# uzh-rpg/rpg_svo

Measured on AMD Instinct MI355X. Metric: frames/sec sparse-align+pose-refine (VGA, 4 pyr lvls); ATE vs CPU ref, higher is better.
Workload: dtype value = default build: K1 f32 pixels/residuals/chi2/per-pixel products, f64 Jacobian rows/partials/reductions/projection/solve/pose; K4 f64 (reference-width build: roofline_f64_build.value)

## Files before the change

include/svo_hip.h:

```cpp
#ifndef SVO_HIP_H_
#define SVO_HIP_H_

#include <stddef.h>
#include <stdint.h>

#ifdef __cplusplus
extern "C" {
#endif

#define SVO_HIP_MAX_LEVELS 8
#define SVO_HIP_STORE_TAIL_PAD 256
#define SVO_HIP_MAX_PATCHES 1024

#define SVO_HIP_OK 0
#define SVO_HIP_EINVAL (-1)
#define SVO_HIP_ERANGE (-2)
#define SVO_HIP_EHIP (-3)
#define SVO_HIP_ENODEV (-4)
#define SVO_HIP_ENOMEM (-5)

#define SVO_HIP_HALFSAMPLE_SCALAR 0
#define SVO_HIP_HALFSAMPLE_SSE2 1
#define SVO_HIP_HALFSAMPLE_AUTO 2

// ... 225 lines not shown
  int32_t* d_visit_cell;
  int32_t* d_visit_trial;
  int32_t* d_trial_cur;
  double* d_trial_pos;
  int32_t* d_trial_obs_begin;
  int32_t* d_trial_obs_end;
  int32_t* d_trial_cell;
  double* d_trial_px;
} svo_hip_reprojection;

int svo_hip_reproject_map(const svo_hip_camera* cam, const svo_hip_frames* frames, int cur_frame,
                          const int32_t* d_kf_rank, const svo_hip_map* map, const svo_hip_map_patch* patch,
                          const svo_hip_grid* grid, int first_cell, int max_cells_with_trials, int max_visits,
                          int max_trials, const svo_hip_reprojection* out, void* stream);

int svo_hip_find_match_direct_indirect(const svo_hip_pyr_layout* layout, const uint8_t* d_store,
                                       const svo_hip_camera* cam, const svo_hip_frames* frames, int M_cap,
                                       const int32_t* d_M, const int32_t* d_cur_frame, const double* d_pt_pos,
                                       const int32_t* d_obs_begin, const int32_t* d_obs_end,
                                       const svo_hip_features* obs, int n_pyr_levels, int align_max_iter,
                                       double* d_px_cur, int32_t* d_ok, int32_t* d_ref_obs, int32_t* d_search_level,
                                       double* d_A_cur_ref, uint8_t* d_patch_out, void* d_workspace,
                                       size_t workspace_bytes, void* stream);
int svo_hip_select_matches_indirect(const svo_hip_camera* cam, int M_cap, const int32_t* d_M, const int32_t* d_cell,
                                    const int32_t* d_ok, const double* d_px, const int32_t* d_level,
                                    const double* d_pos, int max_fts, int32_t* d_n, int32_t* d_sel, double* d_f,
                                    int32_t* d_level_out, double* d_pos_out, uint8_t* d_has_point, int32_t* d_signal,
                                    int32_t signal_value, void* stream);

int svo_hip_compose_poses(int n, const double* d_A, const double* d_B, double* d_out,
                          const int32_t* d_out_index, void* stream);
int svo_hip_cam2world(const svo_hip_camera* cam, int n, const double* d_px, double* d_f,
                      void* stream);
int svo_hip_frame_pose_compose(const double* d_T_cur_ref, const double* d_q_ref, const double* d_t_ref, double* d_frame_T,
                               int cur_frame, double* d_T_copy, double* d_T_out, const svo_hip_camera* cam, int n_frames,
                               int n_kf, const double* d_key_pos, const uint8_t* d_key_valid, int max_n_kfs, int32_t* d_rank,
                               int32_t* d_rank_out, int32_t* d_signal, int32_t signal_value, void* stream);

int svo_hip_pose_optimize(const svo_hip_camera* cam, int B, const int32_t* d_n, int n_stride,
                          const double* d_f, const int32_t* d_level, const double* d_pos,
                          uint8_t* d_has_point, double reproj_thresh, int n_iter,
                          double* d_T_f_w, double* d_Cov, double* d_stats, int32_t* d_ran,
                          void* stream);
int svo_hip_pose_optimize_ordered(const svo_hip_camera* cam, int B, const int32_t* d_n, int n_stride,
                                  const double* d_f, const int32_t* d_level, const double* d_pos,
                                  uint8_t* d_has_point, double reproj_thresh, int n_iter,
                                  double* d_T_f_w, double* d_Cov, double* d_stats, int32_t* d_ran,
                                  void* stream);

int svo_hip_pose_optimize_deferred(const svo_hip_camera* cam, int B, const int32_t* d_n, int n_stride,
                                   const double* d_f, const int32_t* d_level, const double* d_pos,
                                   uint8_t* d_has_point, double reproj_thresh, int n_iter, double* d_T_f_w,
                                   double* d_Cov, double* d_stats, int32_t* d_ran, void* stream);

int svo_hip_point_optimize(const svo_hip_frames* frames, int P, const int32_t* d_obs_ptr,
                           const int32_t* d_obs_frame, const double* d_obs_f, int n_iter,
                           double* d_pos, void* stream);

typedef struct svo_hip_seeds {
  float* d_a;
  float* d_b;
  float* d_mu;
  float* d_z_range;
  float* d_sigma2;
  const int32_t* d_batch_id;
} svo_hip_seeds;

#define SVO_HIP_SEED_ERASED_OLD 1
#define SVO_HIP_SEED_BEHIND 2
#define SVO_HIP_SEED_NOT_IN_FRAME 3
#define SVO_HIP_SEED_NO_MATCH 4
#define SVO_HIP_SEED_UPDATED 5
#define SVO_HIP_SEED_CONVERGED 6
#define SVO_HIP_SEED_NAN 7

typedef struct svo_hip_depth_filter_options {
  int32_t max_n_kfs;
  int32_t batch_counter;
  double seed_convergence_sigma2_thresh;
  int32_t align_1d;
  int32_t align_max_iter;
  int32_t max_epi_search_steps;
  int32_t subpix_refinement;
  int32_t epi_search_edgelet_filtering;
  int32_t n_pyr_levels;
  double epi_search_edgelet_max_angle;
} svo_hip_depth_filter_options;

int svo_hip_update_seeds(const svo_hip_pyr_layout* layout, const uint8_t* d_store,
                         const svo_hip_camera* cam, const svo_hip_frames* frames, int S,
                         const int32_t* d_cur_frame, const svo_hip_features* ftr,
                         const svo_hip_seeds* seeds, const svo_hip_depth_filter_options* opt,
                         int32_t* d_status, double* d_xyz_world, double* d_px_cur,
                         void* d_workspace, size_t workspace_bytes, void* stream);

typedef struct svo_hip_seed_patch {
  int32_t n;
  int32_t reserved;
  const int32_t* d_slot;
  svo_hip_features src_ftr;
  svo_hip_seeds src_seeds;
} svo_hip_seed_patch;
int svo_hip_seed_store_patch(const svo_hip_seed_patch* patch, const svo_hip_features* store_ftr,
                             const svo_hip_seeds* store_seeds, void* stream);
int svo_hip_update_seeds_resident(const svo_hip_pyr_layout* layout, const uint8_t* d_store,
                                  const svo_hip_camera* cam, const svo_hip_frames* frames, int cur_frame, int S,
// ... 184 lines not shown
```

rpg_svo_amd/capi.py:

```python
from __future__ import annotations

import ctypes as C
import os

MAX_LEVELS = 8
STORE_TAIL_PAD = 256
MAX_PATCHES = 1024

HALFSAMPLE_SCALAR, HALFSAMPLE_SSE2, HALFSAMPLE_AUTO = 0, 1, 2
SIA_STOP = 1

_LIB_PATH = os.environ.get("SVO_HIP_LIB") or os.path.join(os.path.dirname(os.path.abspath(__file__)), "lib", "libsvo_hip.so")


class SvoHipError(RuntimeError):
    pass


class PyrLayout(C.Structure):
    _fields_ = [
        ("n_levels", C.c_int32),
        ("w", C.c_int32 * MAX_LEVELS),
        ("h", C.c_int32 * MAX_LEVELS),
        ("pitch", C.c_int32 * MAX_LEVELS),
# ... 156 lines not shown
    "svo_hip_event_sync": (_i, [_vp]),
    "svo_hip_event_query": (_i, [_vp]),
    "svo_hip_stream_wait_event": (_i, [_vp, _vp]),
    "svo_hip_graph_begin_capture": (_i, [_vp]),
    "svo_hip_graph_end_capture": (_i, [_vp, C.POINTER(_vp)]),
    "svo_hip_graph_launch": (_i, [_vp, _vp]),
    "svo_hip_graph_destroy": (_i, [_vp]),
    "svo_hip_camera_pinhole": (_i, [_i, _i] + [C.c_double] * 9 + [C.POINTER(Camera)]),
    "svo_hip_camera_atan": (_i, [_i, _i] + [C.c_double] * 5 + [C.POINTER(Camera)]),
    "svo_hip_pyr_layout_init": (_i, [_i, _i, _i, C.POINTER(PyrLayout)]),
    "svo_hip_pyr_store_bytes": (_i64, [C.POINTER(PyrLayout), _i]),
    "svo_hip_pyramid_load_level0": (_i, [C.POINTER(PyrLayout), _vp, _i, _i, _vp, _i64, _i, _vp]),
    "svo_hip_pyramid_upload_level0": (_i, [C.POINTER(PyrLayout), _vp, _i, _vp, _i, _vp, _vp]),
    "svo_hip_pyramid_upload_level": (_i, [C.POINTER(PyrLayout), _vp, _i, _i, _vp, _i, _vp, _vp]),
    "svo_hip_pyramid_upload_build": (_i, [C.POINTER(PyrLayout), _vp, _i, _vp, _i, _i, _vp, _vp]),
    "svo_hip_pyramid_build": (_i, [C.POINTER(PyrLayout), _vp, _i, _i, _i, _vp]),
    "svo_hip_pyramid_build_from_images": (_i, [C.POINTER(PyrLayout), _vp, _i, _i, _vp, _i64, _i, _i, _vp]),
    "svo_hip_pyramid_build_tiled": (_i, [C.POINTER(PyrLayout), _vp, _i, _i, _vp, _i64, _i, _i, _i, _vp]),
    "svo_hip_pyramid_build_per_level": (_i, [C.POINTER(PyrLayout), _vp, _i, _i, _i, _vp]),
    "svo_hip_pyramid_download_level": (_i, [C.POINTER(PyrLayout), _vp, _i, _i, _vp, _vp]),
    "svo_hip_sparse_align": (_i, [C.POINTER(PyrLayout), _vp, _i, _vp, _vp, _vp, _i, _vp, _vp, _vp,
                                  C.POINTER(SiaParams), _vp, _vp, _vp, _vp, _vp, _vp, _vp, _vp]),
    "svo_hip_sparse_align_workgroup": (_i, [C.POINTER(PyrLayout), _vp, _i, _vp, _vp, _vp, _i, _vp, _vp, _vp,
                                            C.POINTER(SiaParams), _vp, _vp, _vp, _vp, _vp, _vp, _vp, _vp]),
    "svo_hip_solve6_hipsolver_workspace_bytes": (C.c_size_t, [_i]),
    "svo_hip_solve6_hipsolver": (_i, [_i, _vp, _vp, _vp, _vp, _vp, C.c_size_t, _vp]),
    "svo_hip_align_batch": (_i, [_LP, _vp, _i, _vp, _vp, _vp, _vp, _vp, _i, _vp, _vp, _vp, _vp]),
    "svo_hip_align_batch_counted": (_i, [_LP, _vp, _i, _vp, _vp, _vp, _vp, _vp, _i, _vp, _vp, _vp, _vp, _vp]),
    "svo_hip_align_workspace_bytes": (C.c_size_t, [_i]),
    "svo_hip_align_batch_phased": (_i, [_LP, _vp, _i, _vp, _vp, _vp, _vp, _vp, _i, _vp, _vp, _vp, _vp, _vp, C.c_size_t, _vp]),
    "svo_hip_update_seeds_scan_steps": (_vp, [_vp]),
    "svo_hip_update_seeds_count_evaluations": (C.c_int, [C.c_int]),
    "svo_hip_update_seeds_align_evaluations": (_vp, [_vp, C.c_int]),
    "svo_hip_match_workspace_bytes": (C.c_size_t, [_i]),
    "svo_hip_find_match_direct": (_i, [_LP, _vp, C.POINTER(Camera), C.POINTER(Frames), _i, _vp, _vp, _vp,
                                       C.POINTER(Features), _i, _i, _vp, _vp, _vp, _vp, _vp, _vp, _vp, C.c_size_t, _vp]),
    "svo_hip_reproject_map": (_i, [C.POINTER(Camera), C.POINTER(Frames), _i, _vp, C.POINTER(Map), C.POINTER(MapPatch),
                                   C.POINTER(Grid), _i, _i, _i, _i, C.POINTER(Reprojection), _vp]),
    "svo_hip_find_match_direct_indirect": (_i, [_LP, _vp, C.POINTER(Camera), C.POINTER(Frames), _i, _vp, _vp, _vp, _vp, _vp,
                                                C.POINTER(Features), _i, _i, _vp, _vp, _vp, _vp, _vp, _vp, _vp, C.c_size_t, _vp]),
    "svo_hip_select_matches_indirect": (_i, [C.POINTER(Camera), _i, _vp, _vp, _vp, _vp, _vp, _vp, _i, _vp, _vp, _vp, _vp, _vp,
                                             _vp, _vp, _i, _vp]),
    "svo_hip_reproject_points": (_i, [C.POINTER(Camera), C.POINTER(Frames), _i, _vp, _vp, _i, _i, _vp, _vp, _vp]),
    "svo_hip_compose_poses": (_i, [_i, _vp, _vp, _vp, _vp, _vp]),
    "svo_hip_frame_pose_compose": (_i, [_vp, _vp, _vp, _vp, _i, _vp, _vp, _vp, _i, _i, _vp, _vp, _i, _vp, _vp, _vp, _i, _vp]),
    "svo_hip_cam2world": (_i, [C.POINTER(Camera), _i, _vp, _vp, _vp]),
    "svo_hip_select_matches": (_i, [C.POINTER(Camera), _i, _vp, _vp, _vp, _vp, _vp, _i, _vp, _vp, _vp, _vp, _vp, _vp, _vp, _i, _vp]),
    "svo_hip_pose_optimize": (_i, [C.POINTER(Camera), _i, _vp, _i, _vp, _vp, _vp, _vp, C.c_double, _i, _vp, _vp, _vp,
                                   _vp, _vp]),
    "svo_hip_pose_optimize_ordered": (_i, [C.POINTER(Camera), _i, _vp, _i, _vp, _vp, _vp, _vp, C.c_double, _i, _vp, _vp,
                                           _vp, _vp, _vp]),
    "svo_hip_pose_optimize_deferred": (_i, [C.POINTER(Camera), _i, _vp, _i, _vp, _vp, _vp, _vp, C.c_double, _i, _vp, _vp,
                                           _vp, _vp, _vp]),
    "svo_hip_point_optimize": (_i, [C.POINTER(Frames), _i, _vp, _vp, _vp, _i, _vp, _vp]),
    "svo_hip_update_seeds": (_i, [_LP, _vp, C.POINTER(Camera), C.POINTER(Frames), _i, _vp, C.POINTER(Features),
                                  C.POINTER(Seeds), C.POINTER(DepthFilterOptions), _vp, _vp, _vp, _vp, C.c_size_t, _vp]),
    "svo_hip_seed_store_patch": (_i, [C.POINTER(SeedPatch), C.POINTER(Features), C.POINTER(Seeds), _vp]),
    "svo_hip_update_seeds_resident": (_i, [_LP, _vp, C.POINTER(Camera), C.POINTER(Frames), _i, _i, _vp, C.POINTER(Features),
                                           C.POINTER(Seeds), C.POINTER(DepthFilterOptions), _vp, _vp, _vp, _vp, _vp, C.c_size_t, _vp]),
    "svo_hip_update_seeds_resident_pose": (_i, [_LP, _vp, C.POINTER(Camera), C.POINTER(Frames), _i, _vp, _i, _vp, C.POINTER(Features),
                                                C.POINTER(Seeds), C.POINTER(DepthFilterOptions), _vp, _vp, _vp, _vp, _vp, C.c_size_t, _vp]),
    "svo_hip_find_epipolar_match_direct": (_i, [_LP, _vp, C.POINTER(Camera), C.POINTER(Frames), _i, _vp, C.POINTER(Features),
                                                _vp, _vp, _vp, C.POINTER(DepthFilterOptions), _vp, _vp, _vp, _vp, _vp, C.c_size_t, _vp]),
    "svo_hip_update_seed_batch": (_i, [_i, _vp, _vp, C.POINTER(Seeds), _vp]),
    "svo_hip_fast_workspace_bytes": (C.c_size_t, [_LP, _i, _i]),
    "svo_hip_fast_detect": (_i, [_LP, _vp, _i, _vp, _i, _i, _i, _i, _i, _vp, C.c_double, _vp, _vp, _vp, _vp, C.c_size_t, _vp]),
    "svo_hip_klt_params_default": (_i, [C.POINTER(KltParams)]),
    "svo_hip_klt_track": (_i, [_LP, _vp, _i, _vp, _vp, _i, _vp, _vp, _vp, _vp, C.POINTER(KltParams), _vp]),
    "svo_hip_klt_summarize": (_i, [C.POINTER(Camera), _i, _i, _vp, _vp, _vp, _vp, _vp, _vp, _vp, _vp]),
    "svo_hip_homography_params_default": (_i, [C.POINTER(HomographyParams)]),
    "svo_hip_homography_init": (_i, [C.POINTER(Camera), _i, _i, _vp, _vp, _vp, _vp, _vp, _vp, C.POINTER(HomographyParams),
                                     C.POINTER(HomographyOut), _vp]),
    "svo_hip_first_map": (_i, [C.POINTER(Camera), _i, _i, _vp, _vp, _vp, _vp, _vp, _vp, _vp, _vp, _vp, _i, _i, _i, _i,
                               C.POINTER(FirstMapOut), _vp]),
    "svo_hip_initialize_seeds": (_i, [C.POINTER(Camera), _i, _i, _vp, _vp, _vp, C.c_double, _vp, _vp, _vp, _i, _i,
                                      C.POINTER(SeedInitOut), _vp]),
    "svo_hip_frame_close_params_default": (_i, [C.POINTER(FrameCloseParams)]),
    "svo_hip_frame_close": (_i, [C.POINTER(Camera), _i, _i, _i, C.POINTER(FrameCloseIn), _i, _i, _i, _i, C.POINTER(FrameCloseParams),
                                 C.POINTER(FrameCloseOut), _vp]),
    "svo_hip_compute_tau_batch": (_i, [_i, _vp, _vp, _vp, C.c_double, _vp, _vp]),
}

_lib = None


def lib_path() -> str:
    return _LIB_PATH


def load() -> C.CDLL:
    global _lib
    if _lib is not None:
        return _lib
    if not os.path.exists(_LIB_PATH):
        raise SvoHipError(
            f"{_LIB_PATH} not found: build it with `python -c 'import __graft_entry__ as g; g.build()'` "
            "(hipcc --offload-arch=gfx950).  There is no CPU fallback.")
    import torch
    lib = C.CDLL(_LIB_PATH)
    for name, (res, args) in PROTOTYPES.items():
        fn = getattr(lib, name)
        fn.restype = res
        fn.argtypes = args
    _lib = lib
    return lib

# ... 34 lines not shown
```

rpg_svo_amd/csrc/pose_optimizer.hip:

```cpp
#pragma clang fp contract(off)
#include "track_kernels.h"
#include "track_math.h"

using namespace svo_capi;
using namespace svo_dev;

namespace {

constexpr int PO_MINW = 4;
constexpr int PO_HALF = 32;
constexpr int PO_BLOCK = 64;
constexpr int PO_MAXN = 1024;
constexpr double SVO_EPS = 0.0000000001;

struct PoseArgs {
  Cam cam;
  const int32_t* n;
  int n_stride;
  const double* f;
  const int32_t* level;
  const double* pos;
  uint8_t* has_point;
  double reproj_thresh;
  int n_iter;
  double* T;
  double* Cov;
  double* stats;
  int32_t* ran;
  int only_flagged;
};

struct PoseLds {
  double tile[28][PO_HALF];
  unsigned long long live[PO_BLOCK / 64];
  double acc[28];
  double dT[6];
  double new_chi2;
  Se3 T, T_old;
  double scale;
  double median_d;
  double chi2;
  float median_f;
  int n_err;
  int flag;
};

__device__ __forceinline__ float tukey_weight(float x) {
  const float b_square = 4.6851f * 4.6851f;
  const float x_square = x * x;
  if (x_square <= b_square) {
    const float tmp = 1.0f - x_square / b_square;
    return tmp * tmp;
  }
  return 0.0f;
}

template <typename T>
__device__ __forceinline__ void rank_select(const T* v, int n, int k, T* out) {
  for (int i = threadIdx.x; i < n; i += PO_BLOCK) {
    const T mine = v[i];
    if (!(mine < (T)INFINITY)) continue;
    int rank = 0;
#pragma unroll 8
    for (int j = 0; j < n; ++j) {
      const T o = v[j];
      rank += (o < mine || (o == mine && j < i)) ? 1 : 0;
    }
    if (rank == k) *out = mine;
  }
}

struct PoseDyn {
  double* vals;
  float* err;
  uint8_t* hp;
};

__global__ void __launch_bounds__(PO_BLOCK, PO_MINW) pose_opt_kernel(const PoseArgs a) {
  __shared__ PoseLds s;
  SVO_DYNAMIC_LDS(double, po_dyn);
  const int ns8 = (a.n_stride + 7) & ~7;
  PoseDyn d;
  d.vals = po_dyn;
  d.err = reinterpret_cast<float*>(po_dyn + ns8);
  d.hp = reinterpret_cast<uint8_t*>(d.err + ns8);
  const int b = blockIdx.x;
  const int tid = threadIdx.x;
  if (a.only_flagged && a.ran[b] != 2) return;
  int n = a.n[b];
  n = n < 0 ? 0 : (n > a.n_stride ? a.n_stride : n);
  const size_t base = (size_t)b * a.n_stride;
  const double focal = fabs(a.cam.fx);

  if (tid == 0) {
    se3_from_Rt(a.T + 12 * b, s.T);
    s.T_old = s.T;
    s.n_err = 0;
    s.flag = 0;
    s.chi2 = 0.0;
  }
  for (int i = tid; i < n; i += PO_BLOCK) d.hp[i] = a.has_point[base + i];
  __syncthreads();
  {
    const Se3 T = s.T;
    int cnt = 0;
    for (int i = tid; i < n; i += PO_BLOCK) {
      d.err[i] = INFINITY;
      if (!d.hp[i]) continue;
      const double p[3] = {a.pos[3 * (base + i)], a.pos[3 * (base + i) + 1], a.pos[3 * (base + i) + 2]};
      const double fb[3] = {a.f[3 * (base + i)], a.f[3 * (base + i) + 1], a.f[3 * (base + i) + 2]};
      double pf[3], u0[2], u1[2];
      se3_apply(T, p, pf);
      project2d(fb, u0);
      project2d(pf, u1);
      double e[2] = {u0[0] - u1[0], u0[1] - u1[1]};
      const double k = 1.0 / (double)(1 << a.level[base + i]);
      e[0] *= k;
      e[1] *= k;
      d.err[i] = (float)norm2(e);
      ++cnt;
    }
    if (cnt) atomicAdd(&s.n_err, cnt);
  }
  __syncthreads();
  const int n_err = s.n_err;
  if (n_err == 0) {
    if (tid == 0) a.ran[b] = 0;
    return;
  }
  rank_select<float>(d.err, n, n_err / 2, &s.median_f);
  __syncthreads();
  const double estimated_scale = (double)(1.48f * s.median_f);
  if (tid == 0) s.scale = estimated_scale;

  if (tid < 28) s.acc[tid] = 0.0;
  for (int iter = 0; iter < a.n_iter; ++iter) {
    if (tid == 0 && iter == 5) s.scale = 0.85 / focal;
    if (tid < 28) s.acc[tid] = 0.0;
    __syncthreads();
    const Se3 T = s.T;
    const double scale = s.scale;
// ... 147 lines not shown
#pragma unroll
      for (int i = 0; i < 6; ++i) a.Cov[36 * b + i * 6 + tid] = 1.0 * x[i];
    }
  }
  if (tid == 0) se3_to_Rt(s.T, a.T + 12 * b);
  rank_select<double>(d.vals, n, n_err / 2, &s.median_d);
  __syncthreads();
  const double med_init = s.median_d;
  __syncthreads();
  const double reproj_thresh_scaled = a.reproj_thresh / focal;
  {
    const Se3 T = s.T;
    if (tid == 0) s.n_err = 0;
    __syncthreads();
    int deleted = 0;
    for (int i = tid; i < n; i += PO_BLOCK) {
      d.err[i] = 0.f;
      d.vals[i] = INFINITY;
      if (!d.hp[i]) continue;
      const double p[3] = {a.pos[3 * (base + i)], a.pos[3 * (base + i) + 1], a.pos[3 * (base + i) + 2]};
      const double fb[3] = {a.f[3 * (base + i)], a.f[3 * (base + i) + 1], a.f[3 * (base + i) + 2]};
      double pf[3], u0[2], u1[2];
      se3_apply(T, p, pf);
      project2d(fb, u0);
      project2d(pf, u1);
      double e[2] = {u0[0] - u1[0], u0[1] - u1[1]};
      const double k = 1.0 / (double)(1 << a.level[base + i]);
      e[0] *= k;
      e[1] *= k;
      d.vals[i] = e[0] * e[0] + e[1] * e[1];
      d.err[i] = 1.f;
      if (norm2(e) > reproj_thresh_scaled) {
        d.err[i] = 2.f;
        ++deleted;
      }
    }
    if (deleted) atomicAdd(&s.n_err, deleted);
  }
  __syncthreads();
  rank_select<double>(d.vals, n, n_err / 2, &s.median_d);
  __syncthreads();
  const int n_deleted = s.n_err;
  for (int i = tid; i < n; i += PO_BLOCK)
    if (d.err[i] == 2.f) a.has_point[base + i] = 0;
  if (tid == 0) {
    a.stats[4 * b + 0] = estimated_scale * focal;
    a.stats[4 * b + 1] = a.n_iter > 0 ? sqrt(med_init) * focal : 0.0;
    a.stats[4 * b + 2] = sqrt(s.median_d) * focal;
    a.stats[4 * b + 3] = (double)(n_err - n_deleted);
    a.ran[b] = 1;
  }
}

}

static int launch_ordered(const svo_track::PoseWaveArgs& w, int only_flagged, hipStream_t s) {
  PoseArgs a;
  a.cam = make_cam(&w.cam);
  a.n = w.n;
  a.n_stride = w.n_stride;
  a.f = w.f;
  a.level = w.level;
  a.pos = w.pos;
  a.has_point = w.has_point;
  a.reproj_thresh = w.reproj_thresh;
  a.n_iter = w.n_iter;
  a.T = w.T;
  a.Cov = w.Cov;
  a.stats = w.stats;
  a.ran = w.ran;
  a.only_flagged = only_flagged;
  const int ns8 = (w.n_stride + 7) & ~7;
  const size_t dyn = (size_t)ns8 * (sizeof(double) + sizeof(float) + 1);
  hipLaunchKernelGGL(pose_opt_kernel, dim3(w.B), dim3(PO_BLOCK), dyn, s, a);
  return check_launch();
}

enum PoseMode { POSE_WAVE_FINISH, POSE_WAVE_DEFERRED, POSE_ORDERED };

static int pose_optimize_impl(PoseMode mode, const svo_hip_camera* cam, int B, const int32_t* d_n, int n_stride, const double* d_f,
                              const int32_t* d_level, const double* d_pos, uint8_t* d_has_point, double reproj_thresh,
                              int n_iter, double* d_T_f_w, double* d_Cov, double* d_stats, int32_t* d_ran, void* stream) {
  if (!cam || !cam_model_ok(cam) || B < 0 || n_stride < 1 || n_iter < 0) return SVO_HIP_EINVAL;
  if (n_stride > PO_MAXN) return SVO_HIP_ERANGE;
  if (B == 0) return SVO_HIP_OK;
  if (!d_n || !d_f || !d_level || !d_pos || !d_has_point || !d_T_f_w || !d_stats || !d_ran) return SVO_HIP_EINVAL;
  svo_track::PoseWaveArgs w;
  w.cam = *cam;
  w.B = B;
  w.n = d_n;
  w.n_stride = n_stride;
  w.f = d_f;
  w.level = d_level;
  w.pos = d_pos;
  w.has_point = d_has_point;
  w.reproj_thresh = reproj_thresh;
  w.n_iter = n_iter;
  w.T = d_T_f_w;
  w.Cov = d_Cov;
  w.stats = d_stats;
  w.ran = d_ran;
  hipStream_t s = static_cast<hipStream_t>(stream);
  if (mode == POSE_ORDERED || n_stride > svo_track::POSE_WAVE_MAX_STRIDE)
    return launch_ordered(w, 0, s);
  const int rc = svo_track::launch_pose_wave(w, s);
  if (rc != SVO_HIP_OK || mode == POSE_WAVE_DEFERRED) return rc;
  return launch_ordered(w, 1, s);
}

extern "C" int svo_hip_pose_optimize(const svo_hip_camera* cam, int B, const int32_t* d_n, int n_stride,
                                     const double* d_f, const int32_t* d_level, const double* d_pos,
                                     uint8_t* d_has_point, double reproj_thresh, int n_iter, double* d_T_f_w,
                                     double* d_Cov, double* d_stats, int32_t* d_ran, void* stream) {
  return pose_optimize_impl(POSE_WAVE_FINISH, cam, B, d_n, n_stride, d_f, d_level, d_pos, d_has_point, reproj_thresh, n_iter, d_T_f_w,
                            d_Cov, d_stats, d_ran, stream);
}

extern "C" int svo_hip_pose_optimize_deferred(const svo_hip_camera* cam, int B, const int32_t* d_n, int n_stride,
                                              const double* d_f, const int32_t* d_level, const double* d_pos,
                                              uint8_t* d_has_point, double reproj_thresh, int n_iter, double* d_T_f_w,
                                              double* d_Cov, double* d_stats, int32_t* d_ran, void* stream) {
  return pose_optimize_impl(POSE_WAVE_DEFERRED, cam, B, d_n, n_stride, d_f, d_level, d_pos, d_has_point, reproj_thresh, n_iter, d_T_f_w,
                            d_Cov, d_stats, d_ran, stream);
}

extern "C" int svo_hip_pose_optimize_ordered(const svo_hip_camera* cam, int B, const int32_t* d_n, int n_stride,
                                             const double* d_f, const int32_t* d_level, const double* d_pos,
                                             uint8_t* d_has_point, double reproj_thresh, int n_iter, double* d_T_f_w,
                                             double* d_Cov, double* d_stats, int32_t* d_ran, void* stream) {
  return pose_optimize_impl(POSE_ORDERED, cam, B, d_n, n_stride, d_f, d_level, d_pos, d_has_point, reproj_thresh, n_iter, d_T_f_w,
                            d_Cov, d_stats, d_ran, stream);
}
```

rpg_svo_amd/csrc/pose_optimizer_wave.hip:

```cpp
#include "track_kernels.h"
#include "track_math.h"
#include "wave_reduce.h"

using namespace svo_capi;
using namespace svo_dev;

namespace {

using svo_track::PoseWaveArgs;

constexpr int PW_WAVES = 1;
constexpr int PW_MINW = 4;
constexpr double SVO_EPS = 0.0000000001;


__device__ __forceinline__ void uni_se3(Se3& T) {
#pragma unroll
  for (int k = 0; k < 4; ++k) T.q[k] = uniform_f64(T.q[k]);
#pragma unroll
  for (int k = 0; k < 3; ++k) T.t[k] = uniform_f64(T.t[k]);
}


__device__ __forceinline__ double wave_reduce32_f64(const double v[32], int lane) {
  double r[16], q[8], t[4], u[2];
#pragma unroll
  for (int k = 0; k < 16; ++k) r[k] = swap32_add(v[k], v[k + 16]);
#pragma unroll
  for (int k = 0; k < 8; ++k) q[k] = swap16_add(r[k], r[k + 8]);
  {
    const bool hi = (lane & 8) != 0;
#pragma unroll
    for (int k = 0; k < 4; ++k) {
      const double mine = hi ? q[k + 4] : q[k], send = hi ? q[k] : q[k + 4];
      t[k] = mine + dpp_f64<DPP_ROW_ROR8>(send);
    }
  }
  {
    const bool hi = (lane & 4) != 0;
#pragma unroll
    for (int k = 0; k < 2; ++k) {
      const double mine = hi ? t[k + 2] : t[k], send = hi ? t[k] : t[k + 2];
      u[k] = mine + dpp_f64<DPP_ROW_HALF_MIRROR>(send);
    }
  }
  const bool hi = (lane & 2) != 0;
  const double mine = hi ? u[1] : u[0], send = hi ? u[0] : u[1];
  double w = mine + dpp_f64<DPP_QUAD_XOR2>(send);
  w += dpp_f64<DPP_QUAD_XOR1>(w);
  return w;
}

__device__ __forceinline__ double fast_sqrt(double x) {
  const double r = __builtin_amdgcn_rsq(x);
  double g = x * r;
  const double h = 0.5 * r;
  g = fma(fma(-g, g, x), h, g);
  g = fma(fma(-g, g, x), h, g);
  return fmax(g, 0.0);
}

__device__ __forceinline__ void ldlt6_factor_fast(const double H[21], double LD[21]) {
  double d[6];
#pragma unroll
// ... 101 lines not shown
__device__ __forceinline__ bool pivots_ok(const double A[21], const double LD[21]) {
  double dmax = 0.0, imax = 0.0;
  bool zero = false;
#pragma unroll
  for (int k = 0; k < 6; ++k) {
    dmax = fmax(dmax, fabs(A[sym6(k, k)]));
    const double id = fabs(LD[15 + k]);
    zero = zero || !(id > 0.0);
    imax = fmax(imax, id);
  }
  return !zero && (imax * dmax * 1e-9 < 1.0);
}

template <int J>
__device__ __forceinline__ double bcast(double v) { return readlane_f64<2 * J>(v); }

struct PwObs {
  double px, py, pz, ux, uy, k;
};

struct PwBlock {
  double* d;
  float* k;
  uint8_t* slot;
  int cap;
  __device__ __forceinline__ PwObs load(int c) const {
    PwObs o;
    o.px = d[c]; o.py = d[cap + c]; o.pz = d[2 * cap + c]; o.ux = d[3 * cap + c]; o.uy = d[4 * cap + c];
    o.k = (double)k[c];
    return o;
  }
};
constexpr int PW_BYTES_PER_OBS = 5 * 8 + 4 + 1;
__host__ __device__ constexpr int pw_cap(int n_stride) { return (n_stride + 7) & ~7; }

__device__ __forceinline__ double pw_e2(const PwObs& o, const double R[9], const double t[3]) {
  const double x = R[0] * o.px + R[1] * o.py + R[2] * o.pz + t[0];
  const double y = R[3] * o.px + R[4] * o.py + R[5] * o.pz + t[1];
  const double z = R[6] * o.px + R[7] * o.py + R[8] * o.pz + t[2];
  const double zi = fast_rcp(z);
  const double e0 = (o.ux - x * zi) * o.k, e1 = (o.uy - y * zi) * o.k;
  return e0 * e0 + e1 * e1;
}

__device__ __forceinline__ double pw_select(const unsigned long long kd[4], int trips, int k) {
  unsigned long long r;
  if (trips <= 1) r = radix_select<1, unsigned long long>(kd, k, 62);
  else if (trips == 2) r = radix_select<2, unsigned long long>(kd, k, 62);
  else if (trips == 3) r = radix_select<3, unsigned long long>(kd, k, 62);
  else r = radix_select<4, unsigned long long>(kd, k, 62);
  return __longlong_as_double((long long)r);
}

__global__ void __launch_bounds__(64 * PW_WAVES, PW_MINW) pose_opt_wave_kernel(const PoseWaveArgs a) {
  SVO_DYNAMIC_LDS(double, pw_dyn);
  const int lane = threadIdx.x & 63;
  const int wave = threadIdx.x >> 6;
  const int b = blockIdx.x * PW_WAVES + wave;
  if (b >= a.B) return;
  int n = __builtin_amdgcn_readfirstlane(a.n[b]);
  n = n < 0 ? 0 : (n > a.n_stride ? a.n_stride : n);
  const size_t base = (size_t)b * a.n_stride;
  const double focal = fabs(a.cam.fx);

  PwBlock blk;
  blk.cap = pw_cap(a.n_stride);
  blk.d = pw_dyn + (size_t)wave * (blk.cap / 8) * PW_BYTES_PER_OBS;
  blk.k = reinterpret_cast<float*>(blk.d + 5 * blk.cap);
  blk.slot = reinterpret_cast<uint8_t*>(blk.k + blk.cap);
  int n_live = 0;
  for (int j = 0; j * 64 < n; ++j) {
    const int i = j * 64 + lane;
    const bool live = (i < n) && a.has_point[base + i] != 0;
    const unsigned long long m = __ballot(live);
    if (live) {
      const int at = n_live + __popcll(m & ((1ull << lane) - 1ull));
      const int c = at < blk.cap ? at : blk.cap - 1;
      const double* p = a.pos + 3 * (base + i);
      const double* f = a.f + 3 * (base + i);
      blk.d[c] = p[0]; blk.d[blk.cap + c] = p[1]; blk.d[2 * blk.cap + c] = p[2];
      blk.d[3 * blk.cap + c] = f[0] / f[2];
      blk.d[4 * blk.cap + c] = f[1] / f[2];
      blk.k[c] = pow2_inv_f32(a.level[base + i]);
      blk.slot[c] = (uint8_t)i;
    }
    n_live += __popcll(m);
  }
  if (n_live == 0) {
    if (lane == 0) a.ran[b] = 0;
    return;
  }
  SVO_WAVE_LDS_FENCE();
  const int last_pos = (n_live < blk.cap ? n_live : blk.cap) - 1;
  const int trips = (n_live + 63) >> 6;

  Se3 T, T_old;
  se3_from_Rt(a.T + 12 * b, T);
  uni_se3(T);
  T_old = T;
  double R[9];
  quat_to_R(T.q, R);
#pragma unroll
  for (int k = 0; k < 9; ++k) R[k] = uniform_f64(R[k]);

  double estimated_scale, med_init;
  {
    unsigned long long kd[4];
#pragma unroll
    for (int j = 0; j < 4; ++j) {
      kd[j] = 0x7ff0000000000000ull;
      if (j < trips) {
        const int at = j * 64 + lane;
        const double e2 = pw_e2(blk.load(at < last_pos ? at : last_pos), R, T.t);
        if (at < n_live) kd[j] = (unsigned long long)__double_as_longlong(e2);
      }
    }
    med_init = pw_select(kd, trips, n_live / 2);
    const float median_f = (float)sqrt(med_init);
    estimated_scale = (double)(1.48f * median_f);
  }

  double scale = estimated_scale;
  double chi2 = 0.0;
  if (a.n_iter == 0) {
    if (lane == 0) a.ran[b] = 2;
    return;
  }
  for (int iter = 0; iter < a.n_iter; ++iter) {
    if (iter == 5) scale = 0.85 / focal;
    const double inv_scale = 1.0 / scale;
    double A[21];
    double acc[32];
#pragma unroll
    for (int k = 0; k < 32; ++k) acc[k] = 0.0;
#pragma unroll 1
    for (int j = 0; j < trips; ++j) {
      const int at = j * 64 + lane;
      const PwObs o = blk.load(at < last_pos ? at : last_pos);
      const double x = R[0] * o.px + R[1] * o.py + R[2] * o.pz + T.t[0];
      const double y = R[3] * o.px + R[4] * o.py + R[5] * o.pz + T.t[1];
      const double z = R[6] * o.px + R[7] * o.py + R[8] * o.pz + T.t[2];
      const double zi = fast_rcp(z);
      const double xn = x * zi, yn = y * zi;
      const double k = o.k;
      const double e0 = (o.ux - xn) * k, e1 = (o.uy - yn) * k;
      const double e2 = e0 * e0 + e1 * e1;
      const float wf = tukey_w((float)(fast_sqrt(e2) * inv_scale));
      const double w = at < n_live ? (double)wf : 0.0;
      const double j00 = -zi * k, j02 = xn * zi * k, j03 = xn * yn * k, j04 = -(1.0 + xn * xn) * k, j05 = yn * k;
      const double j12 = yn * zi * k, j13 = (1.0 + yn * yn) * k, j14 = -j03, j15 = -xn * k;
// ... 135 lines not shown
```

rpg_svo_amd/csrc/track_kernels.h:

```cpp
#pragma once
#include "capi_common.h"

namespace svo_track {

struct AlignArgs {
  svo_hip_pyr_layout L;
  const uint8_t* store;
  int M;
  const int32_t* slot;
  const int32_t* level;
  const uint8_t* pwb;
  const float* dir;
  const uint8_t* use_1d;
  const uint8_t* active;
  int n_iter;
  const double* px_in;
  double* px_out;
  int scale_out;
  int32_t* ok;
  double* h_inv;
  int32_t* iters = nullptr;
  const int32_t* M_dev = nullptr;
  int it0 = 0, it1 = 1 << 30;
  const int32_t* queue_in = nullptr;
  const int32_t* n_in = nullptr;
  int32_t* queue_out = nullptr;
  int32_t* n_out = nullptr;
  int queue_cap = 0;
  float* state = nullptr;
};
constexpr int ALIGN_NQ = 64;
size_t align_phase_workspace_bytes(int M);
struct SeedArgs;
bool align_takes_finish(int M);
int launch_align(const AlignArgs& a, hipStream_t s, void* d_phase_ws = nullptr, size_t phase_ws_bytes = 0,
                 const SeedArgs* finish = nullptr);

struct WarpArgs {
  svo_hip_pyr_layout L;
  const uint8_t* store;
  int M;
  const uint8_t* active;
  const int32_t* ref_slot;
  const int32_t* ref_level;
  const int32_t* search_level;
  const float* A_ref_cur;
  const float* px_ref_pyr;
  uint8_t* pwb;
  const int32_t* M_dev = nullptr;
};
int launch_warp(const WarpArgs& a, hipStream_t s);

struct PoseWaveArgs {
  svo_hip_camera cam;
  int B;
  const int32_t* n;
  int n_stride;
  const double* f;
  const int32_t* level;
  const double* pos;
  uint8_t* has_point;
  double reproj_thresh;
  int n_iter;
  double* T;
  double* Cov;
  double* stats;
  int32_t* ran;
};
constexpr int POSE_WAVE_MAX_STRIDE = 256;
int launch_pose_wave(const PoseWaveArgs& a, hipStream_t s);

struct Carver {
  uint8_t* p;
  size_t left;
  bool ok = true;
  Carver(void* base, size_t bytes) : p(static_cast<uint8_t*>(base)), left(bytes) {}
  template <typename T>
  T* take(size_t n) {
    const size_t need = (n * sizeof(T) + 255) & ~size_t(255);
    if (need > left) { ok = false; return nullptr; }
    T* r = reinterpret_cast<T*>(p);
    p += need;
    left -= need;
    return r;
  }
  static size_t round(size_t n_bytes) { return (n_bytes + 255) & ~size_t(255); }
};

}
```

rpg_svo_amd/tracking.py:

```python
from __future__ import annotations

import ctypes as C
from dataclasses import dataclass

import torch

from . import capi
from .pyramid import PyramidStore, _stream_ptr


def _ptr(t):
    return None if t is None else t.data_ptr()


def _chk(t, dtype):
    assert t.is_cuda and t.dtype == dtype and t.is_contiguous(), "device-resident contiguous tensor required"
    return t


class FrameTable:

    def __init__(self, slot: torch.Tensor, T_f_w: torch.Tensor):
        self.slot = _chk(slot, torch.int32)
        self.T_f_w = _chk(T_f_w, torch.float64)
# ... 143 lines not shown
    capi.check(lib.svo_hip_compose_poses(n, _chk(A, torch.float64).data_ptr(), _chk(B, torch.float64).data_ptr(),
                                         _chk(out, torch.float64).data_ptr(), _ptr(out_index), _stream_ptr(A.device)),
               "svo_hip_compose_poses")
    return out


def cam2world(cam, px, out=None):
    lib = capi.load()
    n = px.shape[0]
    if out is None:
        out = torch.empty(n, 3, dtype=torch.float64, device=px.device)
    c = capi.camera(cam)
    capi.check(lib.svo_hip_cam2world(C.byref(c), n, _chk(px, torch.float64).data_ptr(), out.data_ptr(),
                                     _stream_ptr(px.device)), "svo_hip_cam2world")
    return out


def select_matches(cam, cell, ok, px, level, pos, max_fts):
    lib = capi.load()
    M = cell.shape[0]
    dev = px.device
    cap = max(1, min(M, max_fts + 1))
    n = torch.zeros(1, dtype=torch.int32, device=dev)
    sel = torch.full((cap,), -1, dtype=torch.int32, device=dev)
    f = torch.zeros(cap, 3, dtype=torch.float64, device=dev)
    level_out = torch.zeros(cap, dtype=torch.int32, device=dev)
    pos_out = torch.zeros(cap, 3, dtype=torch.float64, device=dev)
    has_point = torch.zeros(cap, dtype=torch.uint8, device=dev)
    c = capi.camera(cam)
    capi.check(lib.svo_hip_select_matches(C.byref(c), M, _chk(cell, torch.int32).data_ptr(), _chk(ok, torch.int32).data_ptr(),
                                          _chk(px, torch.float64).data_ptr(), _chk(level, torch.int32).data_ptr(),
                                          _chk(pos, torch.float64).data_ptr(), int(max_fts), n.data_ptr(), sel.data_ptr(),
                                          f.data_ptr(), level_out.data_ptr(), pos_out.data_ptr(), has_point.data_ptr(),
                                          None, 0, _stream_ptr(dev)), "svo_hip_select_matches")
    return n, sel, f, level_out, pos_out, has_point


@dataclass
class PoseOptResult:
    T_f_w: torch.Tensor
    Cov: torch.Tensor
    stats: torch.Tensor
    ran: torch.Tensor
    has_point: torch.Tensor


def optimize_gauss_newton(cam, n, f, level, pos, has_point, T_f_w, reproj_thresh: float = 2.0, n_iter: int = 10,
                          ordered: bool = False, out: PoseOptResult | None = None, deferred: bool = False) -> PoseOptResult:
    lib = capi.load()
    B, ns = f.shape[0], f.shape[1]
    dev = f.device
    _chk(n, torch.int32); _chk(f, torch.float64); _chk(level, torch.int32); _chk(pos, torch.float64)
    _chk(has_point, torch.uint8); _chk(T_f_w, torch.float64)
    if out is not None:
        res = out
        res.T_f_w.copy_(T_f_w)
        res.has_point.copy_(has_point)
    else:
        res = PoseOptResult(T_f_w.clone(), torch.zeros(B, 36, dtype=torch.float64, device=dev),
                            torch.zeros(B, 4, dtype=torch.float64, device=dev), torch.zeros(B, dtype=torch.int32, device=dev),
                            has_point.clone())
    c = capi.camera(cam)
    fn = lib.svo_hip_pose_optimize_ordered if ordered else (lib.svo_hip_pose_optimize_deferred if deferred else lib.svo_hip_pose_optimize)
    capi.check(fn(C.byref(c), B, n.data_ptr(), ns, f.data_ptr(), level.data_ptr(), pos.data_ptr(),
                  res.has_point.data_ptr(), reproj_thresh, n_iter, res.T_f_w.data_ptr(),
                  res.Cov.data_ptr(), res.stats.data_ptr(), res.ran.data_ptr(), _stream_ptr(dev)),
               "svo_hip_pose_optimize")
    return res


@dataclass
class FrameClose:
    gate: torch.Tensor
    quality: torch.Tensor
    result: torch.Tensor
    T_out: torch.Tensor
    nobs_out: torch.Tensor
    depth_mean: torch.Tensor
    depth_min: torch.Tensor
    kf_block: torch.Tensor
    valid: torch.Tensor
    xyz_ref: torch.Tensor
    key_pts: torch.Tensor
    occupancy: torch.Tensor
    kf_remove: torch.Tensor


_FRAME_CLOSE_DTYPES = dict(gate=torch.int32, quality=torch.int32, result=torch.int32, T_out=torch.float64, nobs_out=torch.int32,
                           depth_mean=torch.float64, depth_min=torch.float64, kf_block=torch.int32, valid=torch.uint8,
                           xyz_ref=torch.float64, key_pts=torch.int32, occupancy=torch.uint8, kf_remove=torch.int32)


def frame_close_outputs(B: int, n_stride: int, cells: int, device) -> FrameClose:
    shape = dict(T_out=(B, 12), valid=(B, n_stride), xyz_ref=(B, n_stride, 3), key_pts=(B, 5), occupancy=(B, cells))
    return FrameClose(**{k: torch.zeros(shape.get(k, (B,)), dtype=dt, device=device) for k, dt in _FRAME_CLOSE_DTYPES.items()})


def frame_close_params(**fields) -> capi.FrameCloseParams:
    p = capi.FrameCloseParams()
    capi.check(capi.load().svo_hip_frame_close_params_default(C.byref(p)), "svo_hip_frame_close_params_default")
    for k, v in fields.items():
        assert k in dict(capi.FrameCloseParams._fields_) and k != "reserved", k
        setattr(p, k, v)
    return p


def close_frame(cam, n, px, f, pos, has_point, T_f_w, T_last, num_obs, num_obs_last, n_kf, kf_T, kf_overlap, cell_size: int,
                grid_n_cols: int, grid_n_rows: int, params: capi.FrameCloseParams | None = None,
                out: FrameClose | None = None) -> FrameClose:
    B, ns = has_point.shape
    nk = kf_overlap.shape[1]
    i32, f64 = torch.int32, torch.float64
    for t, dt, shape in ((n, i32, (B,)), (px, f64, (B, ns, 2)), (f, f64, (B, ns, 3)), (pos, f64, (B, ns, 3)), (has_point, torch.uint8, (B, ns)),
                         (T_f_w, f64, (B, 12)), (T_last, f64, (B, 12)), (num_obs, i32, (B,)), (num_obs_last, i32, (B,)), (n_kf, i32, (B,)),
                         (kf_T, f64, (B, nk, 12)), (kf_overlap, i32, (B, nk))):
# ... 212 lines not shown
```

Measured before the change: 12.50 million.

## Fuse pose input copies into wave kernel and compact flagged-frame fallback launch

Adds a pose_optimize_into entry point that reads has_point and T from input buffers and writes them to output buffers inside the wave kernel. This removes the two separate torch copy kernels when an output struct is reused. The wave kernel's gather loop is restructured to issue all loads up front across fixed trips before writing to LDS. The flagged fallback now launches one workgroup per 64 frames and loops over the flagged ones found by a ballot, instead of one workgroup per frame that mostly exits early. The cost is a fixed-trip, register-heavy load phase and serialized fallback frames within a workgroup.

```diff
diff --git a/include/svo_hip.h b/include/svo_hip.h
--- a/include/svo_hip.h
+++ b/include/svo_hip.h
@@ -301,6 +301,11 @@
                                    const double* d_f, const int32_t* d_level, const double* d_pos,
                                    uint8_t* d_has_point, double reproj_thresh, int n_iter, double* d_T_f_w,
                                    double* d_Cov, double* d_stats, int32_t* d_ran, void* stream);
+
+int svo_hip_pose_optimize_into(const svo_hip_camera* cam, int B, const int32_t* d_n, int n_stride, const double* d_f,
+                               const int32_t* d_level, const double* d_pos, const uint8_t* d_has_point_in,
+                               const double* d_T_in, double reproj_thresh, int n_iter, uint8_t* d_has_point_out,
+                               double* d_T_out, double* d_Cov, double* d_stats, int32_t* d_ran, void* stream);
 
 int svo_hip_point_optimize(const svo_hip_frames* frames, int P, const int32_t* d_obs_ptr,
                            const int32_t* d_obs_frame, const double* d_obs_f, int n_iter,
diff --git a/rpg_svo_amd/capi.py b/rpg_svo_amd/capi.py
--- a/rpg_svo_amd/capi.py
+++ b/rpg_svo_amd/capi.py
@@ -232,6 +232,8 @@
                                            _vp, _vp, _vp]),
     "svo_hip_pose_optimize_deferred": (_i, [C.POINTER(Camera), _i, _vp, _i, _vp, _vp, _vp, _vp, C.c_double, _i, _vp, _vp,
                                            _vp, _vp, _vp]),
+    "svo_hip_pose_optimize_into": (_i, [C.POINTER(Camera), _i, _vp, _i, _vp, _vp, _vp, _vp, _vp, C.c_double, _i, _vp, _vp, _vp,
+                                        _vp, _vp, _vp]),
     "svo_hip_point_optimize": (_i, [C.POINTER(Frames), _i, _vp, _vp, _vp, _i, _vp, _vp]),
     "svo_hip_update_seeds": (_i, [_LP, _vp, C.POINTER(Camera), C.POINTER(Frames), _i, _vp, C.POINTER(Features),
                                   C.POINTER(Seeds), C.POINTER(DepthFilterOptions), _vp, _vp, _vp, _vp, C.c_size_t, _vp]),
diff --git a/rpg_svo_amd/csrc/pose_optimizer.hip b/rpg_svo_amd/csrc/pose_optimizer.hip
--- a/rpg_svo_amd/csrc/pose_optimizer.hip
+++ b/rpg_svo_amd/csrc/pose_optimizer.hip
@@ -10,6 +10,7 @@
 constexpr int PO_MINW = 4;
 constexpr int PO_HALF = 32;
 constexpr int PO_BLOCK = 64;
+static_assert(PO_BLOCK == 64, "pose_opt_flagged_kernel finds its frames with one ballot over the workgroup");
 constexpr int PO_MAXN = 1024;
 constexpr double SVO_EPS = 0.0000000001;
 
@@ -27,7 +28,7 @@
   double* Cov;
   double* stats;
   int32_t* ran;
-  int only_flagged;
+  int B;
 };
 
 struct PoseLds {
@@ -76,17 +77,8 @@
   uint8_t* hp;
 };
 
-__global__ void __launch_bounds__(PO_BLOCK, PO_MINW) pose_opt_kernel(const PoseArgs a) {
-  __shared__ PoseLds s;
-  SVO_DYNAMIC_LDS(double, po_dyn);
-  const int ns8 = (a.n_stride + 7) & ~7;
-  PoseDyn d;
-  d.vals = po_dyn;
-  d.err = reinterpret_cast<float*>(po_dyn + ns8);
-  d.hp = reinterpret_cast<uint8_t*>(d.err + ns8);
-  const int b = blockIdx.x;
+__device__ __forceinline__ void pose_opt_frame(const PoseArgs& a, const int b, PoseLds& s, const PoseDyn& d) {
   const int tid = threadIdx.x;
-  if (a.only_flagged && a.ran[b] != 2) return;
   int n = a.n[b];
   n = n < 0 ? 0 : (n > a.n_stride ? a.n_stride : n);
   const size_t base = (size_t)b * a.n_stride;
@@ -340,6 +332,36 @@
   }
 }
 
+__device__ __forceinline__ PoseDyn pose_dyn(double* po_dyn, int n_stride) {
+  const int ns8 = (n_stride + 7) & ~7;
+  PoseDyn d;
+  d.vals = po_dyn;
+  d.err = reinterpret_cast<float*>(po_dyn + ns8);
+  d.hp = reinterpret_cast<uint8_t*>(d.err + ns8);
+  return d;
+}
+
+__global__ void __launch_bounds__(PO_BLOCK, PO_MINW) pose_opt_kernel(const PoseArgs a) {
+  __shared__ PoseLds s;
+  SVO_DYNAMIC_LDS(double, po_dyn);
+  pose_opt_frame(a, blockIdx.x, s, pose_dyn(po_dyn, a.n_stride));
+}
+
+__global__ void __launch_bounds__(PO_BLOCK, PO_MINW) pose_opt_flagged_kernel(const PoseArgs a) {
+  __shared__ PoseLds s;
+  SVO_DYNAMIC_LDS(double, po_dyn);
+  const PoseDyn d = pose_dyn(po_dyn, a.n_stride);
+  const int b0 = blockIdx.x * PO_BLOCK;
+  const int mine = b0 + (int)threadIdx.x;
+  unsigned long long todo = __ballot(mine < a.B && a.ran[mine] == 2);
+  while (todo) {
+    const int k = __ffsll((long long)todo) - 1;
+    todo &= todo - 1;
+    pose_opt_frame(a, b0 + k, s, d);
+    __syncthreads();
+  }
+}
+
 }
 
 static int launch_ordered(const svo_track::PoseWaveArgs& w, int only_flagged, hipStream_t s) {
@@ -357,22 +379,27 @@
   a.Cov = w.Cov;
   a.stats = w.stats;
   a.ran = w.ran;
-  a.only_flagged = only_flagged;
+  a.B = w.B;
   const int ns8 = (w.n_stride + 7) & ~7;
   const size_t dyn = (size_t)ns8 * (sizeof(double) + sizeof(float) + 1);
-  hipLaunchKernelGGL(pose_opt_kernel, dim3(w.B), dim3(PO_BLOCK), dyn, s, a);
+  if (only_flagged)
+    hipLaunchKernelGGL(pose_opt_flagged_kernel, dim3((w.B + PO_BLOCK - 1) / PO_BLOCK), dim3(PO_BLOCK), dyn, s, a);
+  else
+    hipLaunchKernelGGL(pose_opt_kernel, dim3(w.B), dim3(PO_BLOCK), dyn, s, a);
   return check_launch();
 }
 
 enum PoseMode { POSE_WAVE_FINISH, POSE_WAVE_DEFERRED, POSE_ORDERED };
 
 static int pose_optimize_impl(PoseMode mode, const svo_hip_camera* cam, int B, const int32_t* d_n, int n_stride, const double* d_f,
-                              const int32_t* d_level, const double* d_pos, uint8_t* d_has_point, double reproj_thresh,
-                              int n_iter, double* d_T_f_w, double* d_Cov, double* d_stats, int32_t* d_ran, void* stream) {
+                              const int32_t* d_level, const double* d_pos, const uint8_t* d_has_point_in, uint8_t* d_has_point,
+                              double reproj_thresh, int n_iter, const double* d_T_in, double* d_T_f_w, double* d_Cov,
+                              double* d_stats, int32_t* d_ran, void* stream) {
   if (!cam || !cam_model_ok(cam) || B < 0 || n_stride < 1 || n_iter < 0) return SVO_HIP_EINVAL;
   if (n_stride > PO_MAXN) return SVO_HIP_ERANGE;
   if (B == 0) return SVO_HIP_OK;
-  if (!d_n || !d_f || !d_level || !d_pos || !d_has_point || !d_T_f_w || !d_stats || !d_ran) return SVO_HIP_EINVAL;
+  if (!d_n || !d_f || !d_level || !d_pos || !d_has_point_in || !d_has_point || !d_T_in || !d_T_f_w || !d_stats || !d_ran)
+    return SVO_HIP_EINVAL;
   svo_track::PoseWaveArgs w;
   w.cam = *cam;
   w.B = B;
@@ -381,16 +408,22 @@
   w.f = d_f;
   w.level = d_level;
   w.pos = d_pos;
+  w.has_point_in = d_has_point_in;
   w.has_point = d_has_point;
   w.reproj_thresh = reproj_thresh;
   w.n_iter = n_iter;
+  w.T_in = d_T_in;
   w.T = d_T_f_w;
   w.Cov = d_Cov;
   w.stats = d_stats;
   w.ran = d_ran;
   hipStream_t s = static_cast<hipStream_t>(stream);
-  if (mode == POSE_ORDERED || n_stride > svo_track::POSE_WAVE_MAX_STRIDE)
+  if (mode == POSE_ORDERED || n_stride > svo_track::POSE_WAVE_MAX_STRIDE) {
+    if (d_has_point_in != d_has_point)
+      SVO_HIP_TRY(hipMemcpyAsync(d_has_point, d_has_point_in, (size_t)B * n_stride, hipMemcpyDeviceToDevice, s));
+    if (d_T_in != d_T_f_w) SVO_HIP_TRY(hipMemcpyAsync(d_T_f_w, d_T_in, (size_t)B * 12 * sizeof(double), hipMemcpyDeviceToDevice, s));
     return launch_ordered(w, 0, s);
+  }
   const int rc = svo_track::launch_pose_wave(w, s);
   if (rc != SVO_HIP_OK || mode == POSE_WAVE_DEFERRED) return rc;
   return launch_ordered(w, 1, s);
@@ -400,22 +433,30 @@
                                      const double* d_f, const int32_t* d_level, const double* d_pos,
                                      uint8_t* d_has_point, double reproj_thresh, int n_iter, double* d_T_f_w,
                                      double* d_Cov, double* d_stats, int32_t* d_ran, void* stream) {
-  return pose_optimize_impl(POSE_WAVE_FINISH, cam, B, d_n, n_stride, d_f, d_level, d_pos, d_has_point, reproj_thresh, n_iter, d_T_f_w,
-                            d_Cov, d_stats, d_ran, stream);
+  return pose_optimize_impl(POSE_WAVE_FINISH, cam, B, d_n, n_stride, d_f, d_level, d_pos, d_has_point, d_has_point, reproj_thresh, n_iter,
+                            d_T_f_w, d_T_f_w, d_Cov, d_stats, d_ran, stream);
 }
 
 extern "C" int svo_hip_pose_optimize_deferred(const svo_hip_camera* cam, int B, const int32_t* d_n, int n_stride,
                                               const double* d_f, const int32_t* d_level, const double* d_pos,
                                               uint8_t* d_has_point, double reproj_thresh, int n_iter, double* d_T_f_w,
                                               double* d_Cov, double* d_stats, int32_t* d_ran, void* stream) {
-  return pose_optimize_impl(POSE_WAVE_DEFERRED, cam, B, d_n, n_stride, d_f, d_level, d_pos, d_has_point, reproj_thresh, n_iter, d_T_f_w,
-                            d_Cov, d_stats, d_ran, stream);
+  return pose_optimize_impl(POSE_WAVE_DEFERRED, cam, B, d_n, n_stride, d_f, d_level, d_pos, d_has_point, d_has_point, reproj_thresh, n_iter,
+                            d_T_f_w, d_T_f_w, d_Cov, d_stats, d_ran, stream);
 }
 
 extern "C" int svo_hip_pose_optimize_ordered(const svo_hip_camera* cam, int B, const int32_t* d_n, int n_stride,
                                              const double* d_f, const int32_t* d_level, const double* d_pos,
                                              uint8_t* d_has_point, double reproj_thresh, int n_iter, double* d_T_f_w,
                                              double* d_Cov, double* d_stats, int32_t* d_ran, void* stream) {
-  return pose_optimize_impl(POSE_ORDERED, cam, B, d_n, n_stride, d_f, d_level, d_pos, d_has_point, reproj_thresh, n_iter, d_T_f_w,
-                            d_Cov, d_stats, d_ran, stream);
-}
+  return pose_optimize_impl(POSE_ORDERED, cam, B, d_n, n_stride, d_f, d_level, d_pos, d_has_point, d_has_point, reproj_thresh, n_iter,
+                            d_T_f_w, d_T_f_w, d_Cov, d_stats, d_ran, stream);
+}
+
+extern "C" int svo_hip_pose_optimize_into(const svo_hip_camera* cam, int B, const int32_t* d_n, int n_stride, const double* d_f,
+                                          const int32_t* d_level, const double* d_pos, const uint8_t* d_has_point_in,
+                                          const double* d_T_in, double reproj_thresh, int n_iter, uint8_t* d_has_point_out,
+                                          double* d_T_out, double* d_Cov, double* d_stats, int32_t* d_ran, void* stream) {
+  return pose_optimize_impl(POSE_WAVE_FINISH, cam, B, d_n, n_stride, d_f, d_level, d_pos, d_has_point_in, d_has_point_out, reproj_thresh,
+                            n_iter, d_T_in, d_T_out, d_Cov, d_stats, d_ran, stream);
+}
diff --git a/rpg_svo_amd/csrc/pose_optimizer_wave.hip b/rpg_svo_amd/csrc/pose_optimizer_wave.hip
--- a/rpg_svo_amd/csrc/pose_optimizer_wave.hip
+++ b/rpg_svo_amd/csrc/pose_optimizer_wave.hip
@@ -10,6 +10,7 @@
 using svo_track::PoseWaveArgs;
 
 constexpr int PW_WAVES = 1;
+constexpr int PW_TRIPS = svo_track::POSE_WAVE_MAX_STRIDE / 64;
 constexpr int PW_MINW = 4;
 constexpr double SVO_EPS = 0.0000000001;
 
@@ -217,11 +218,17 @@
   return __longlong_as_double((long long)r);
 }
 
+__device__ __forceinline__ void pw_loads_done() {
+#ifdef __HIP_DEVICE_COMPILE__
+  __builtin_amdgcn_s_waitcnt(0x0F70);
+#endif
+}
+
 __global__ void __launch_bounds__(64 * PW_WAVES, PW_MINW) pose_opt_wave_kernel(const PoseWaveArgs a) {
   SVO_DYNAMIC_LDS(double, pw_dyn);
   const int lane = threadIdx.x & 63;
   const int wave = threadIdx.x >> 6;
-  const int b = blockIdx.x * PW_WAVES + wave;
+  const int b = __builtin_amdgcn_readfirstlane(blockIdx.x * PW_WAVES + wave);
   if (b >= a.B) return;
   int n = __builtin_amdgcn_readfirstlane(a.n[b]);
   n = n < 0 ? 0 : (n > a.n_stride ? a.n_stride : n);
@@ -233,23 +240,56 @@
   blk.d = pw_dyn + (size_t)wave * (blk.cap / 8) * PW_BYTES_PER_OBS;
   blk.k = reinterpret_cast<float*>(blk.d + 5 * blk.cap);
   blk.slot = reinterpret_cast<uint8_t*>(blk.k + blk.cap);
+  const bool carry = a.has_point_in != a.has_point;
+  uint8_t flag[PW_TRIPS];
+#pragma unroll
+  for (int j = 0; j < PW_TRIPS; ++j) {
+    const int i = j * 64 + lane;
+    flag[j] = a.has_point_in[base + (i < a.n_stride ? i : a.n_stride - 1)];
+  }
+  pw_loads_done();
+  bool live[PW_TRIPS];
+  int at[PW_TRIPS];
   int n_live = 0;
-  for (int j = 0; j * 64 < n; ++j) {
-    const int i = j * 64 + lane;
-    const bool live = (i < n) && a.has_point[base + i] != 0;
-    const unsigned long long m = __ballot(live);
-    if (live) {
-      const int at = n_live + __popcll(m & ((1ull << lane) - 1ull));
-      const int c = at < blk.cap ? at : blk.cap - 1;
-      const double* p = a.pos + 3 * (base + i);
-      const double* f = a.f + 3 * (base + i);
-      blk.d[c] = p[0]; blk.d[blk.cap + c] = p[1]; blk.d[2 * blk.cap + c] = p[2];
-      blk.d[3 * blk.cap + c] = f[0] / f[2];
-      blk.d[4 * blk.cap + c] = f[1] / f[2];
-      blk.k[c] = pow2_inv_f32(a.level[base + i]);
-      blk.slot[c] = (uint8_t)i;
-    }
+#pragma unroll
+  for (int j = 0; j < PW_TRIPS; ++j) {
+    live[j] = (j * 64 + lane < n) && flag[j] != 0;
+    const unsigned long long m = __ballot(live[j]);
+    const int c = n_live + __popcll(m & ((1ull << lane) - 1ull));
+    at[j] = c < blk.cap ? c : blk.cap - 1;
     n_live += __popcll(m);
+  }
+  double p[PW_TRIPS][3], f[PW_TRIPS][3];
+  int lv[PW_TRIPS];
+#pragma unroll
+  for (int j = 0; j < PW_TRIPS; ++j) {
+    const size_t src = base + (live[j] ? j * 64 + lane : 0);
+#pragma unroll
+    for (int k = 0; k < 3; ++k) p[j][k] = a.pos[3 * src + k];
+#pragma unroll
+    for (int k = 0; k < 3; ++k) f[j][k] = a.f[3 * src + k];
+    lv[j] = a.level[src];
+  }
+  const double t_raw = a.T_in[12 * b + (lane < 12 ? lane : 11)];
+  pw_loads_done();
+  if (a.T_in != a.T && lane < 12) a.T[12 * b + lane] = t_raw;
+  if (carry) {
+#pragma unroll
+    for (int j = 0; j < PW_TRIPS; ++j) {
+      const int i = j * 64 + lane;
+      if (i < a.n_stride) a.has_point[base + i] = flag[j];
+    }
+  }
+#pragma unroll
+  for (int j = 0; j < PW_TRIPS; ++j) {
+    if (live[j]) {
+      const int c = at[j];
+      blk.d[c] = p[j][0]; blk.d[blk.cap + c] = p[j][1]; blk.d[2 * blk.cap + c] = p[j][2];
+      blk.d[3 * blk.cap + c] = f[j][0] / f[j][2];
+      blk.d[4 * blk.cap + c] = f[j][1] / f[j][2];
+      blk.k[c] = pow2_inv_f32(lv[j]);
+      blk.slot[c] = (uint8_t)(j * 64 + lane);
+    }
   }
   if (n_live == 0) {
     if (lane == 0) a.ran[b] = 0;
@@ -260,7 +300,12 @@
   const int trips = (n_live + 63) >> 6;
 
   Se3 T, T_old;
-  se3_from_Rt(a.T + 12 * b, T);
+  {
+    const double Rt[12] = {readlane_f64<0>(t_raw), readlane_f64<1>(t_raw), readlane_f64<2>(t_raw),  readlane_f64<3>(t_raw),
+                           readlane_f64<4>(t_raw), readlane_f64<5>(t_raw), readlane_f64<6>(t_raw),  readlane_f64<7>(t_raw),
+                           readlane_f64<8>(t_raw), readlane_f64<9>(t_raw), readlane_f64<10>(t_raw), readlane_f64<11>(t_raw)};
+    se3_from_Rt(Rt, T);
+  }
   uni_se3(T);
   T_old = T;
   double R[9];
diff --git a/rpg_svo_amd/csrc/track_kernels.h b/rpg_svo_amd/csrc/track_kernels.h
--- a/rpg_svo_amd/csrc/track_kernels.h
+++ b/rpg_svo_amd/csrc/track_kernels.h
@@ -59,9 +59,11 @@
   const double* f;
   const int32_t* level;
   const double* pos;
+  const uint8_t* has_point_in;
   uint8_t* has_point;
   double reproj_thresh;
   int n_iter;
+  const double* T_in;
   double* T;
   double* Cov;
   double* stats;
diff --git a/rpg_svo_amd/tracking.py b/rpg_svo_amd/tracking.py
--- a/rpg_svo_amd/tracking.py
+++ b/rpg_svo_amd/tracking.py
@@ -219,6 +219,16 @@
     dev = f.device
     _chk(n, torch.int32); _chk(f, torch.float64); _chk(level, torch.int32); _chk(pos, torch.float64)
     _chk(has_point, torch.uint8); _chk(T_f_w, torch.float64)
+    c = capi.camera(cam)
+    if out is not None and not (ordered or deferred):
+        _chk(out.has_point, torch.uint8); _chk(out.T_f_w, torch.float64)
+        assert out.has_point.numel() == has_point.numel() == B * ns and out.T_f_w.numel() == T_f_w.numel() == 12 * B
+        capi.check(lib.svo_hip_pose_optimize_into(C.byref(c), B, n.data_ptr(), ns, f.data_ptr(), level.data_ptr(), pos.data_ptr(),
+                                                  has_point.data_ptr(), T_f_w.data_ptr(), reproj_thresh, n_iter,
+                                                  out.has_point.data_ptr(), out.T_f_w.data_ptr(), out.Cov.data_ptr(),
+                                                  out.stats.data_ptr(), out.ran.data_ptr(), _stream_ptr(dev)),
+                   "svo_hip_pose_optimize_into")
+        return out
     if out is not None:
         res = out
         res.T_f_w.copy_(T_f_w)
@@ -227,7 +237,6 @@
         res = PoseOptResult(T_f_w.clone(), torch.zeros(B, 36, dtype=torch.float64, device=dev),
                             torch.zeros(B, 4, dtype=torch.float64, device=dev), torch.zeros(B, dtype=torch.int32, device=dev),
                             has_point.clone())
-    c = capi.camera(cam)
     fn = lib.svo_hip_pose_optimize_ordered if ordered else (lib.svo_hip_pose_optimize_deferred if deferred else lib.svo_hip_pose_optimize)
     capi.check(fn(C.byref(c), B, n.data_ptr(), ns, f.data_ptr(), level.data_ptr(), pos.data_ptr(),
                   res.has_point.data_ptr(), reproj_thresh, n_iter, res.T_f_w.data_ptr(),
```

Result: faster. 12.65 million (median of 6 runs) (+1.2%).
